# hustvl/4DGaussians

Hardware: NVIDIA H100
Metric: render FPS @300k gauss 1352x1014 (fused deform+rasterize forward); train-step ms in `train_step` (higher is better)
Workload: dtype f32

## Files before the change

### 4dgaussians_b200/csrc/g4d_deform_tc.cu

```cuda
#include "geom_finish.cuh"
#include "tc_wgmma.cuh"

namespace g4d {

template <int ARITH> struct TcArith;
template <> struct TcArith<2> {
    static constexpr int KS = 16, ES = 2, EPC = 8, NWG = 2, PH = 1;
    static constexpr float SF = 64.f, SA = 8.f, SW = 256.f;
};
template <> struct TcArith<1> {
    static constexpr int KS = 8, ES = 4, EPC = 4, NWG = 1, PH = 4;
    static constexpr float SF = 1.f, SA = 1.f, SW = 1.f;
};
constexpr float kF16Max = 65504.f;
constexpr int kStageCols = 60;
constexpr uint32_t kMaxSmemPerBlock = 227u * 1024u;
constexpr uint32_t kTcStaticSmem = (uint32_t)((sizeof(CameraDev) + 127) & ~(size_t)127);

struct TcSmem { uint32_t w1, w0, w2, bias, w2s, stage, bars, part_bytes, total; };

inline TcSmem tc_smem_layout(int arith, int F, bool sh) {
    const uint32_t es = arith == 2 ? 2u : 4u, ph = arith == 2 ? 1u : 4u, nwg = arith == 2 ? 2u : 1u;
    TcSmem s{};
    uint32_t off = 0;
// ... 99 lines not shown

template <int ARITH, int N, int NS, int NSP>
__device__ __forceinline__ void gemm3(float (&d)[N / 2], const Frags<NS>& a, int s0, uint32_t b_hi, uint32_t b_lo, uint32_t bcols,
                                      bool accumulate) {
    using A = TcArith<ARITH>;
    const uint64_t dh = wg::desc_kmajor(b_hi, bcols, A::EPC), dl = wg::desc_kmajor(b_lo, bcols, A::EPC);
    wg::fence_regs(d);
    wg::fence();
#pragma unroll
    for (int p = 0; p < 3; ++p) {
#pragma unroll
        for (int s = 0; s < NSP; ++s) {
            const uint64_t bd = ((p == 1) ? dl : dh) + (uint64_t)(16 * s);
            const uint32_t acc = (accumulate || p > 0 || s > 0) ? 1u : 0u;
            if constexpr (ARITH == 2) wg::mma_f16_rs<N, 0>(d, p == 0 ? a.lo[s0 + s] : a.hi[s0 + s], bd, acc);
            else wg::mma_tf32_rs<N>(d, p == 0 ? a.lo[s0 + s] : a.hi[s0 + s], bd, acc);
        }
    }
    wg::commit();
    wg::wait_all();
    wg::fence_regs(d);
}

template <int ARITH>
__device__ __forceinline__ void relu_to_frags(const float (&d)[64], float inv, const float* __restrict__ bias, int t, Frags<128 / TcArith<ARITH>::KS>& a,
                                              uint32_t (&b0)[4], uint32_t (&b1)[4], float& mx) {
#pragma unroll
    for (int w = 0; w < 4; ++w) { b0[w] = 0u; b1[w] = 0u; }
#pragma unroll
    for (int j = 0; j < 16; ++j) {
        const int c = 8 * j + 2 * t;
        const float2 bb = *reinterpret_cast<const float2*>(bias + c);
        const float x0 = fmaf(d[4 * j], inv, bb.x), x1 = fmaf(d[4 * j + 1], inv, bb.y);
        const float y0 = fmaf(d[4 * j + 2], inv, bb.x), y1 = fmaf(d[4 * j + 3], inv, bb.y);
        const int sh = 8 * (j & 3) + 2 * t;
        b0[j >> 2] |= ((x0 > 0.f ? 1u : 0u) | (x1 > 0.f ? 2u : 0u)) << sh;
        b1[j >> 2] |= ((y0 > 0.f ? 1u : 0u) | (y1 > 0.f ? 2u : 0u)) << sh;
        const float r0 = fmaxf(x0, 0.f), r1 = fmaxf(x1, 0.f), r2 = fmaxf(y0, 0.f), r3 = fmaxf(y1, 0.f);
        mx = fmaxf(mx, fmaxf(fmaxf(r0, r1), fmaxf(r2, r3)));
        put_block<ARITH>(a, j, r0, r1, r2, r3);
    }
#pragma unroll
    for (int w = 0; w < 4; ++w) {
        b0[w] |= __shfl_xor_sync(0xffffffffu, b0[w], 1); b0[w] |= __shfl_xor_sync(0xffffffffu, b0[w], 2);
        b1[w] |= __shfl_xor_sync(0xffffffffu, b1[w], 1); b1[w] |= __shfl_xor_sync(0xffffffffu, b1[w], 2);
    }
}

__device__ __forceinline__ void store_bits(uint32_t* base, int slot, int64_t n, int64_t g0, int64_t g1, int t, const uint32_t (&b0)[4],
                                           const uint32_t (&b1)[4]) {
    const uint32_t w0 = t == 0 ? b0[0] : t == 1 ? b0[1] : t == 2 ? b0[2] : b0[3];
    const uint32_t w1 = t == 0 ? b1[0] : t == 1 ? b1[1] : t == 2 ? b1[2] : b1[3];
    if (g0 < n) base[((size_t)slot * (size_t)n + (size_t)g0) * 4 + t] = w0;
    if (g1 < n) base[((size_t)slot * (size_t)n + (size_t)g1) * 4 + t] = w1;
}

__device__ __forceinline__ void mbar_arrive(void* bar) {
    asm volatile("mbarrier.arrive.shared::cta.b64 _, [%0];" ::"r"(smem_u32(bar)) : "memory");
}
__device__ __forceinline__ void bar_sync(int id, int count) { asm volatile("bar.sync %0, %1;" ::"r"(id), "r"(count) : "memory"); }

template <int ARITH, int MODE, int C, int L, bool SAVE>
__global__ void __launch_bounds__(TcArith<ARITH>::NWG * 128, 1)
deform_tc_kernel(DeformDesc d, TcWeights tw, TcSmem Ls, const CameraDev* __restrict__ camp, int use_cam, int64_t n, DeformIO io) {
    using A = TcArith<ARITH>;
    constexpr int F = C * L, NS0 = F / A::KS, NS1 = 128 / A::KS, NSP = NS1 / A::PH, TM = 64 * A::NWG, NT = 128 * A::NWG;
    static_assert(F % 16 == 0 && F <= 64, "feature width must be 32, 48 or 64");
    constexpr float kInvL0 = A::SA / (A::SF * A::SW), kInvH = 1.f / (A::SA * A::SW), kInvHS = 1.f / A::SW;
// ... 42 lines not shown
    uint32_t hseq = 0;
    {
        int k = 0;
        for (int h = 0; h < G4D_NUM_HEADS; ++h)
            if (d.head_mask & (1 << h)) hseq |= (uint32_t)h << (3 * k++);
    }
    const int64_t ntiles = (n + TM - 1) / TM;
    const int64_t my_tiles = (int64_t)blockIdx.x < ntiles ? (ntiles - 1 - blockIdx.x) / gridDim.x + 1 : 0;
    const uint32_t per_tile = (uint32_t)(m_heads * A::PH), total_items = (uint32_t)my_tiles * per_tile;
    auto issue = [&](uint32_t u) {
        const uint32_t s = u & 1u, r = u % per_tile;
        if (u >= 2) mbar_wait(bar_empty + s, ((u >> 1) - 1u) & 1u);
        const int h = (int)((hseq >> (3 * (r / A::PH))) & 7u);
        mbar_expect_tx(bar_full + s, Ls.part_bytes);
        tma_bulk_g2s(smem + Ls.w1 + s * Ls.part_bytes, reinterpret_cast<const uint8_t*>(tw.w1[h]) + (r % A::PH) * Ls.part_bytes,
                     Ls.part_bytes, bar_full + s);
    };
    if (tid == 0) {
        const uint32_t w0b = 2u * 128u * F * A::ES, w2b = hsh ? 2u * 48u * 128u * A::ES : 0u;
        mbar_expect_tx(bar_w0, w0b + w2b);
        tma_bulk_g2s(smem + Ls.w0, tw.w0, w0b, bar_w0);
        if (hsh) tma_bulk_g2s(smem + Ls.w2, tw.w2[4], w2b, bar_w0);
        if (total_items) issue(0);
    }
    __syncwarp();
    mbar_wait(bar_w0, 0);
    const uint32_t sW0 = wg::smem_addr(smem + Ls.w0), sW1 = wg::smem_addr(smem + Ls.w1), sW2 = wg::smem_addr(smem + Ls.w2);
    const float* b2s = sBias + 128 + G4D_NUM_HEADS * 128;
    float mx = 0.f;
    uint32_t u = 0;
    const bool dbg = tw.dbg && tid == 0;
    const long long t_start = dbg ? clock64() : 0;
    long long t_wait = 0;

    for (int64_t it = 0; it < my_tiles; ++it) {
        const int64_t tile = (int64_t)blockIdx.x + it * gridDim.x;
        const int64_t row0 = tile * TM + wgi * 64, g0 = row0 + r0, g1 = row0 + r1;
        float acc[64];
        {
            Frags<NS0> x;
            const float* f0 = tw.feat + g0 * F;
            const float* f1 = tw.feat + g1 * F;
#pragma unroll
            for (int s = 0; s < NS0; ++s) {
                float v[8];
#pragma unroll
                for (int hlf = 0; hlf < 2; ++hlf) {
                    const int c = ARITH == 2 ? 16 * s + 8 * hlf + 2 * t : 8 * s + 4 * hlf + t;
                    if (ARITH == 2) {
                        const float2 p0 = g0 < n ? __ldg(reinterpret_cast<const float2*>(f0 + c)) : make_float2(0.f, 0.f);
                        const float2 p1 = g1 < n ? __ldg(reinterpret_cast<const float2*>(f1 + c)) : make_float2(0.f, 0.f);
                        v[4 * hlf] = p0.x * A::SF; v[4 * hlf + 1] = p0.y * A::SF; v[4 * hlf + 2] = p1.x * A::SF; v[4 * hlf + 3] = p1.y * A::SF;
                    } else {
                        v[4 * hlf] = g0 < n ? __ldg(f0 + c) : 0.f;
                        v[4 * hlf + 2] = g1 < n ? __ldg(f1 + c) : 0.f;
                    }
                }
                if (ARITH == 2) {
#pragma unroll
                    for (int e = 0; e < 8; ++e) mx = fmaxf(mx, fabsf(v[e]));
                    wg::f16_split2(v[0], v[1], x.hi[s][0], x.lo[s][0]);
                    wg::f16_split2(v[2], v[3], x.hi[s][1], x.lo[s][1]);
                    wg::f16_split2(v[4], v[5], x.hi[s][2], x.lo[s][2]);
                    wg::f16_split2(v[6], v[7], x.hi[s][3], x.lo[s][3]);
                } else {
                    wg::tf32_split(v[0], x.hi[s][0], x.lo[s][0]);
                    wg::tf32_split(v[2], x.hi[s][1], x.lo[s][1]);
                    wg::tf32_split(v[4], x.hi[s][2], x.lo[s][2]);
                    wg::tf32_split(v[6], x.hi[s][3], x.lo[s][3]);
                }
            }
            gemm3<ARITH, 128, NS0, NS0>(acc, x, 0, sW0, sW0 + 128u * F * A::ES, F, false);
        }
        Frags<NS1> a1;
        {
            uint32_t bw0[4], bw1[4];
            relu_to_frags<ARITH>(acc, kInvL0, sBias, t, a1, bw0, bw1, mx);
            if (SAVE) store_bits(tw.relu_bits, 0, n, g0, g1, t, bw0, bw1);
        }
        if (t == 0) {
#pragma unroll
            for (int j = 0; j < 11; ++j) { stage[r0 * kStageCols + j] = 0.f; stage[r1 * kStageCols + j] = 0.f; }
        }
#pragma unroll 1
        for (int k = 0; k < m_heads; ++k) {
            const int h = (int)((hseq >> (3 * k)) & 7u);
#pragma unroll 1
            for (int p = 0; p < A::PH; ++p, ++u) {
                if (tid == 0 && u + 1 < total_items) issue(u + 1);
                __syncwarp();
                const uint32_t s = u & 1u;
                const long long t0 = dbg ? clock64() : 0;
                mbar_wait(bar_full + s, (u >> 1) & 1u);
                if (dbg) t_wait += clock64() - t0;
                const uint32_t b = sW1 + s * Ls.part_bytes;
                if constexpr (A::PH == 1) {
                    gemm3<ARITH, 128, NS1, NSP>(acc, a1, 0, b, b + Ls.part_bytes / 2, 128 / A::PH, false);
                } else {
#pragma unroll
                    for (int pp = 0; pp < A::PH; ++pp)
                        if (pp == p) gemm3<ARITH, 128, NS1, NSP>(acc, a1, pp * NSP, b, b + Ls.part_bytes / 2, 128 / A::PH, pp != 0);
                }
                if (lane == 0) mbar_arrive(bar_empty + s);
            }
            uint32_t bw0[4], bw1[4];
            if (h < 4) {
                const float* b1 = sBias + 128 + h * 128;
                const float4* w2 = sW2s + h * 128;
                float o0[4] = {0.f, 0.f, 0.f, 0.f}, o1[4] = {0.f, 0.f, 0.f, 0.f};
#pragma unroll
                for (int w = 0; w < 4; ++w) { bw0[w] = 0u; bw1[w] = 0u; }
#pragma unroll
                for (int j = 0; j < 16; ++j) {
                    const int c = 8 * j + 2 * t;
                    const float2 bb = *reinterpret_cast<const float2*>(b1 + c);
                    const float x0 = fmaf(acc[4 * j], kInvH, bb.x), x1 = fmaf(acc[4 * j + 1], kInvH, bb.y);
                    const float y0 = fmaf(acc[4 * j + 2], kInvH, bb.x), y1 = fmaf(acc[4 * j + 3], kInvH, bb.y);
                    const int sh = 8 * (j & 3) + 2 * t;
                    bw0[j >> 2] |= ((x0 > 0.f ? 1u : 0u) | (x1 > 0.f ? 2u : 0u)) << sh;
                    bw1[j >> 2] |= ((y0 > 0.f ? 1u : 0u) | (y1 > 0.f ? 2u : 0u)) << sh;
                    const float4 wa = w2[c], wb = w2[c + 1];
                    const float ax = fmaxf(x0, 0.f), ay = fmaxf(x1, 0.f), bx = fmaxf(y0, 0.f), by = fmaxf(y1, 0.f);
                    o0[0] = fmaf(ay, wb.x, fmaf(ax, wa.x, o0[0])); o0[1] = fmaf(ay, wb.y, fmaf(ax, wa.y, o0[1]));
                    o0[2] = fmaf(ay, wb.z, fmaf(ax, wa.z, o0[2])); o0[3] = fmaf(ay, wb.w, fmaf(ax, wa.w, o0[3]));
                    o1[0] = fmaf(by, wb.x, fmaf(bx, wa.x, o1[0])); o1[1] = fmaf(by, wb.y, fmaf(bx, wa.y, o1[1]));
                    o1[2] = fmaf(by, wb.z, fmaf(bx, wa.z, o1[2])); o1[3] = fmaf(by, wb.w, fmaf(bx, wa.w, o1[3]));
                }
#pragma unroll
                for (int o = 0; o < 4; ++o) {
                    o0[o] += __shfl_xor_sync(0xffffffffu, o0[o], 1); o0[o] += __shfl_xor_sync(0xffffffffu, o0[o], 2);
                    o1[o] += __shfl_xor_sync(0xffffffffu, o1[o], 1); o1[o] += __shfl_xor_sync(0xffffffffu, o1[o], 2);
                }
#pragma unroll
                for (int w = 0; w < 4; ++w) {
                    bw0[w] |= __shfl_xor_sync(0xffffffffu, bw0[w], 1); bw0[w] |= __shfl_xor_sync(0xffffffffu, bw0[w], 2);
                    bw1[w] |= __shfl_xor_sync(0xffffffffu, bw1[w], 1); bw1[w] |= __shfl_xor_sync(0xffffffffu, bw1[w], 2);
                }
                if (t == 0) {
                    const int ko = head_out(h), col = head_col(h);
#pragma unroll
                    for (int o = 0; o < 4; ++o) {
                        if (o < ko) {
                            stage[r0 * kStageCols + col + o] = o0[o] + b2s[4 * h + o];
                            stage[r1 * kStageCols + col + o] = o1[o] + b2s[4 * h + o];
                        }
                    }
                }
            } else {
                relu_to_frags<ARITH>(acc, kInvHS, sBias + 128 + 4 * 128, t, a1, bw0, bw1, mx);
                float acc2[24];
                gemm3<ARITH, 48, NS1, NS1>(acc2, a1, 0, sW2, sW2 + 48u * 128u * A::ES, 128, false);
                const float* b2sh = b2s + 16;
#pragma unroll
                for (int j = 0; j < 6; ++j) {
                    const int c = 8 * j + 2 * t;
                    stage[r0 * kStageCols + 11 + c] = fmaf(acc2[4 * j], kInvH, b2sh[c]);
                    stage[r0 * kStageCols + 12 + c] = fmaf(acc2[4 * j + 1], kInvH, b2sh[c + 1]);
                    stage[r1 * kStageCols + 11 + c] = fmaf(acc2[4 * j + 2], kInvH, b2sh[c]);
                    stage[r1 * kStageCols + 12 + c] = fmaf(acc2[4 * j + 3], kInvH, b2sh[c + 1]);
                }
            }
            if (SAVE) store_bits(tw.relu_bits, 1 + h, n, g0, g1, t, bw0, bw1);
        }
        bar_sync(1 + wgi, 128);
        {
            const int row = t128 & 63;
            const int64_t gi = row0 + row;
            const float* o = stage + row * kStageCols;
            if (gi < n) {
                const Vec3 p{io.xyz[3 * gi] + o[0], io.xyz[3 * gi + 1] + o[1], io.xyz[3 * gi + 2] + o[2]};
                if (t128 < 64) {
                    float sl[3] = {0.f, 0.f, 0.f}, q[4] = {0.f, 0.f, 0.f, 0.f}, ol = 0.f;
                    if (io.scaling) { sl[0] = io.scaling[3 * gi]; sl[1] = io.scaling[3 * gi + 1]; sl[2] = io.scaling[3 * gi + 2]; }
                    if (io.rotation) { const float4 r4 = *reinterpret_cast<const float4*>(io.rotation + 4 * gi); q[0] = r4.x; q[1] = r4.y; q[2] = r4.z; q[3] = r4.w; }
                    if (io.opacity) ol = io.opacity[gi];
                    sl[0] += o[3]; sl[1] += o[4]; sl[2] += o[5];
                    q[0] += o[6]; q[1] += o[7]; q[2] += o[8]; q[3] += o[9];
                    ol += o[10];
                    if (MODE == 0) {
                        io.out_xyz[3 * gi] = p.x; io.out_xyz[3 * gi + 1] = p.y; io.out_xyz[3 * gi + 2] = p.z;
                        if (io.out_scaling) { io.out_scaling[3 * gi] = sl[0]; io.out_scaling[3 * gi + 1] = sl[1]; io.out_scaling[3 * gi + 2] = sl[2]; }
                        if (io.out_rotation) *reinterpret_cast<float4*>(io.out_rotation + 4 * gi) = make_float4(q[0], q[1], q[2], q[3]);
                        if (io.out_opacity) io.out_opacity[gi] = ol;
                    } else {
                        fused_finish_geometry(cam, io, gi, p, sl, q, ol);
                    }
                } else {
                    float dsh[48];
#pragma unroll
                    for (int j = 0; j < 48; ++j) dsh[j] = hsh ? o[11 + j] : 0.f;
                    if (MODE == 0) {
                        if (io.out_shs && hsh) {
#pragma unroll
                            for (int j = 0; j < 48; j += 4) {
                                const float4 b = *reinterpret_cast<const float4*>(io.shs + gi * 48 + j);
                                *reinterpret_cast<float4*>(io.out_shs + gi * 48 + j) = make_float4(b.x + dsh[j], b.y + dsh[j + 1], b.z + dsh[j + 2], b.w + dsh[j + 3]);
                            }
                        }
                    } else {
                        fused_finish_colour(cam, io, gi, p, hsh, dsh);
                    }
                }
            }
        }
        bar_sync(1 + wgi, 128);
    }
    if (ARITH == 2 && mx >= kF16Max && tw.status) *reinterpret_cast<volatile uint32_t*>(tw.status) = 1u;
    if (dbg) { tw.dbg[blockIdx.x * 12] = clock64() - t_start; tw.dbg[blockIdx.x * 12 + 1] = t_wait; }
}

template <int C4>
__global__ void __launch_bounds__(256) deform_features_kernel(DeformDesc d, int64_t n, const float* __restrict__ xyz, float* __restrict__ feat) {
    pdl_wait();
    pdl_trigger();
    const int64_t t = (int64_t)blockIdx.x * 256 + threadIdx.x;
    const int64_t g = t / C4;
    const int v = (int)(t % C4);
    if (g >= n) return;
    const AabbNorm nrm(d.aabb);
    float pcs[3];
#pragma unroll
    for (int a = 0; a < 3; ++a) pcs[a] = nrm(a, xyz[3 * g + a]);
    for (int l = 0; l < d.levels; ++l) {
        Tap1D tx[3];
#pragma unroll
        for (int a = 0; a < 3; ++a) tx[a] = make_tap(pcs[a], d.res[l][a]);
        *reinterpret_cast<float4*>(feat + g * d.F + l * d.C + 4 * v) = sample_vector(d.planes[l], d.trow[l], d.res[l], tx, v, C4);
    }
}

cudaError_t launch_deform_features(const DeformDesc& d, int64_t n, const float* xyz, float* feat, bool pdl, cudaStream_t st) {
// ... 59 lines not shown
```

### 4dgaussians_b200/csrc/tc_wgmma.cuh

```cuda
#pragma once
#include <cuda_runtime.h>
#include <stdint.h>

namespace g4d {
namespace wg {

__device__ __forceinline__ uint32_t smem_addr(const void* p) { return (uint32_t)__cvta_generic_to_shared(p); }

__device__ __forceinline__ uint64_t make_desc(uint32_t saddr, uint32_t lbo_bytes, uint32_t sbo_bytes) {
    return (uint64_t)((saddr >> 4) & 0x3FFFu) | ((uint64_t)((lbo_bytes >> 4) & 0x3FFFu) << 16) |
           ((uint64_t)((sbo_bytes >> 4) & 0x3FFFu) << 32);
}
__device__ __forceinline__ uint64_t desc_kmajor(uint32_t saddr, uint32_t cols, uint32_t elems_per_core) {
    return make_desc(saddr, 128u, (cols / elems_per_core) * 128u);
}
__device__ __forceinline__ uint64_t desc_mnmajor(uint32_t saddr, uint32_t cols) { return make_desc(saddr, (cols / 8u) * 128u, 128u); }

__host__ __device__ constexpr uint32_t img16_off(uint32_t row, uint32_t col, uint32_t ncols) {
    return (row >> 3) * ((ncols >> 3) * 128u) + (col >> 3) * 128u + (row & 7u) * 16u + (col & 7u) * 2u;
}
__host__ __device__ constexpr uint32_t img32_off(uint32_t row, uint32_t col, uint32_t ncols) {
    return (row >> 3) * ((ncols >> 2) * 128u) + (col >> 2) * 128u + (row & 7u) * 16u + (col & 3u) * 4u;
}
__host__ __device__ constexpr uint32_t tf32_kperm(uint32_t c) { return (c & ~7u) | ((c & 1u) ? 4u + ((c & 7u) >> 1) : ((c & 7u) >> 1)); }

__device__ __forceinline__ void fence() { asm volatile("wgmma.fence.sync.aligned;" ::: "memory"); }
__device__ __forceinline__ void commit() { asm volatile("wgmma.commit_group.sync.aligned;" ::: "memory"); }
__device__ __forceinline__ void wait_all() { asm volatile("wgmma.wait_group.sync.aligned 0;" ::: "memory"); }
__device__ __forceinline__ void fence_proxy_async() { asm volatile("fence.proxy.async.shared::cta;" ::: "memory"); }
template <int M>
__device__ __forceinline__ void fence_regs(float (&d)[M]) {
#pragma unroll
    for (int i = 0; i < M; ++i) asm volatile("" : "+f"(d[i])::"memory");
}
template <int M>
__device__ __forceinline__ void fence_regs(uint32_t (&d)[M]) {
#pragma unroll
    for (int i = 0; i < M; ++i) asm volatile("" : "+r"(d[i])::"memory");
}

__device__ __forceinline__ uint32_t tf32_rna(float x) {
    uint32_t r;
    asm("cvt.rna.tf32.f32 %0, %1;" : "=r"(r) : "f"(x));
    return r;
}
__device__ __forceinline__ void tf32_split(float x, uint32_t& hi, uint32_t& lo) {
    hi = tf32_rna(x);
    lo = tf32_rna(x - __uint_as_float(hi));
}
__device__ __forceinline__ uint16_t bf16_rn(float x) {
    uint16_t r;
// ... 15 lines not shown
    asm("{\n\t.reg .b16 l, h;\n\tmov.b32 {l, h}, %2;\n\tcvt.f32.f16 %0, l;\n\tcvt.f32.f16 %1, h;\n\t}" : "=f"(ha), "=f"(hb) : "r"(hi));
    asm("cvt.rn.satfinite.f16x2.f32 %0, %1, %2;" : "=r"(lo) : "f"(b - hb), "f"(a - ha));
}

template <int NS>
struct Frags { uint32_t hi[NS][4], lo[NS][4]; };


__device__ __forceinline__ void mma_tf32_rs_n16(float (&d)[8], const uint32_t (&a)[4], uint64_t b, uint32_t acc) {
    asm volatile(
        "{\n.reg .pred p;\nsetp.ne.b32 p, %13, 0;\n"
        "wgmma.mma_async.sync.aligned.m64n16k8.f32.tf32.tf32 {%0, %1, %2, %3, %4, %5, %6, %7}, {%8, %9, %10, %11}, %12, p, 1, 1;\n}\n"
        : "+f"(d[0]), "+f"(d[1]), "+f"(d[2]), "+f"(d[3]), "+f"(d[4]), "+f"(d[5]), "+f"(d[6]), "+f"(d[7])
        : "r"(a[0]), "r"(a[1]), "r"(a[2]), "r"(a[3]), "l"(b), "r"(acc));
}

__device__ __forceinline__ void mma_tf32_rs_n48(float (&d)[24], const uint32_t (&a)[4], uint64_t b, uint32_t acc) {
    asm volatile(
        "{\n.reg .pred p;\nsetp.ne.b32 p, %29, 0;\n"
        "wgmma.mma_async.sync.aligned.m64n48k8.f32.tf32.tf32 {%0, %1, %2, %3, %4, %5, %6, %7, %8, %9, %10, %11, %12, %13, %14, %15, %16, %17, %18, %19, %20, %21, %22, %23}, {%24, %25, %26, %27}, %28, p, 1, 1;\n}\n"
        : "+f"(d[0]), "+f"(d[1]), "+f"(d[2]), "+f"(d[3]), "+f"(d[4]), "+f"(d[5]), "+f"(d[6]), "+f"(d[7]),
          "+f"(d[8]), "+f"(d[9]), "+f"(d[10]), "+f"(d[11]), "+f"(d[12]), "+f"(d[13]), "+f"(d[14]), "+f"(d[15]),
          "+f"(d[16]), "+f"(d[17]), "+f"(d[18]), "+f"(d[19]), "+f"(d[20]), "+f"(d[21]), "+f"(d[22]), "+f"(d[23])
        : "r"(a[0]), "r"(a[1]), "r"(a[2]), "r"(a[3]), "l"(b), "r"(acc));
}

__device__ __forceinline__ void mma_tf32_rs_n128(float (&d)[64], const uint32_t (&a)[4], uint64_t b, uint32_t acc) {
    asm volatile(
        "{\n.reg .pred p;\nsetp.ne.b32 p, %69, 0;\n"
        "wgmma.mma_async.sync.aligned.m64n128k8.f32.tf32.tf32 {%0, %1, %2, %3, %4, %5, %6, %7, %8, %9, %10, %11, %12, %13, %14, %15, %16, %17, %18, %19, %20, %21, %22, %23, %24, %25, %26, %27, %28, %29, %30, %31, %32, %33, %34, %35, %36, %37, %38, %39, %40, %41, %42, %43, %44, %45, %46, %47, %48, %49, %50, %51, %52, %53, %54, %55, %56, %57, %58, %59, %60, %61, %62, %63}, {%64, %65, %66, %67}, %68, p, 1, 1;\n}\n"
        : "+f"(d[0]), "+f"(d[1]), "+f"(d[2]), "+f"(d[3]), "+f"(d[4]), "+f"(d[5]), "+f"(d[6]), "+f"(d[7]),
          "+f"(d[8]), "+f"(d[9]), "+f"(d[10]), "+f"(d[11]), "+f"(d[12]), "+f"(d[13]), "+f"(d[14]), "+f"(d[15]),
          "+f"(d[16]), "+f"(d[17]), "+f"(d[18]), "+f"(d[19]), "+f"(d[20]), "+f"(d[21]), "+f"(d[22]), "+f"(d[23]),
          "+f"(d[24]), "+f"(d[25]), "+f"(d[26]), "+f"(d[27]), "+f"(d[28]), "+f"(d[29]), "+f"(d[30]), "+f"(d[31]),
          "+f"(d[32]), "+f"(d[33]), "+f"(d[34]), "+f"(d[35]), "+f"(d[36]), "+f"(d[37]), "+f"(d[38]), "+f"(d[39]),
          "+f"(d[40]), "+f"(d[41]), "+f"(d[42]), "+f"(d[43]), "+f"(d[44]), "+f"(d[45]), "+f"(d[46]), "+f"(d[47]),
          "+f"(d[48]), "+f"(d[49]), "+f"(d[50]), "+f"(d[51]), "+f"(d[52]), "+f"(d[53]), "+f"(d[54]), "+f"(d[55]),
          "+f"(d[56]), "+f"(d[57]), "+f"(d[58]), "+f"(d[59]), "+f"(d[60]), "+f"(d[61]), "+f"(d[62]), "+f"(d[63])
        : "r"(a[0]), "r"(a[1]), "r"(a[2]), "r"(a[3]), "l"(b), "r"(acc));
}

template <int N>
__device__ __forceinline__ void mma_tf32_rs(float (&d)[N / 2], const uint32_t (&a)[4], uint64_t b, uint32_t acc) {
    static_assert(N == 16 || N == 48 || N == 128, "unsupported N");
    if constexpr (N == 16) mma_tf32_rs_n16(d, a, b, acc);
    else if constexpr (N == 48) mma_tf32_rs_n48(d, a, b, acc);
    else if constexpr (N == 128) mma_tf32_rs_n128(d, a, b, acc);
}

template <int TB>
__device__ __forceinline__ void mma_f16_rs_n16(float (&d)[8], const uint32_t (&a)[4], uint64_t b, uint32_t acc) {
    asm volatile(
        "{\n.reg .pred p;\nsetp.ne.b32 p, %13, 0;\n"
        "wgmma.mma_async.sync.aligned.m64n16k16.f32.f16.f16 {%0, %1, %2, %3, %4, %5, %6, %7}, {%8, %9, %10, %11}, %12, p, 1, 1, %14;\n}\n"
        : "+f"(d[0]), "+f"(d[1]), "+f"(d[2]), "+f"(d[3]), "+f"(d[4]), "+f"(d[5]), "+f"(d[6]), "+f"(d[7])
        : "r"(a[0]), "r"(a[1]), "r"(a[2]), "r"(a[3]), "l"(b), "r"(acc), "n"(TB));
}

template <int TB>
__device__ __forceinline__ void mma_f16_rs_n48(float (&d)[24], const uint32_t (&a)[4], uint64_t b, uint32_t acc) {
    asm volatile(
        "{\n.reg .pred p;\nsetp.ne.b32 p, %29, 0;\n"
        "wgmma.mma_async.sync.aligned.m64n48k16.f32.f16.f16 {%0, %1, %2, %3, %4, %5, %6, %7, %8, %9, %10, %11, %12, %13, %14, %15, %16, %17, %18, %19, %20, %21, %22, %23}, {%24, %25, %26, %27}, %28, p, 1, 1, %30;\n}\n"
        : "+f"(d[0]), "+f"(d[1]), "+f"(d[2]), "+f"(d[3]), "+f"(d[4]), "+f"(d[5]), "+f"(d[6]), "+f"(d[7]),
          "+f"(d[8]), "+f"(d[9]), "+f"(d[10]), "+f"(d[11]), "+f"(d[12]), "+f"(d[13]), "+f"(d[14]), "+f"(d[15]),
          "+f"(d[16]), "+f"(d[17]), "+f"(d[18]), "+f"(d[19]), "+f"(d[20]), "+f"(d[21]), "+f"(d[22]), "+f"(d[23])
        : "r"(a[0]), "r"(a[1]), "r"(a[2]), "r"(a[3]), "l"(b), "r"(acc), "n"(TB));
}

template <int TB>
__device__ __forceinline__ void mma_f16_rs_n128(float (&d)[64], const uint32_t (&a)[4], uint64_t b, uint32_t acc) {
    asm volatile(
        "{\n.reg .pred p;\nsetp.ne.b32 p, %69, 0;\n"
        "wgmma.mma_async.sync.aligned.m64n128k16.f32.f16.f16 {%0, %1, %2, %3, %4, %5, %6, %7, %8, %9, %10, %11, %12, %13, %14, %15, %16, %17, %18, %19, %20, %21, %22, %23, %24, %25, %26, %27, %28, %29, %30, %31, %32, %33, %34, %35, %36, %37, %38, %39, %40, %41, %42, %43, %44, %45, %46, %47, %48, %49, %50, %51, %52, %53, %54, %55, %56, %57, %58, %59, %60, %61, %62, %63}, {%64, %65, %66, %67}, %68, p, 1, 1, %70;\n}\n"
        : "+f"(d[0]), "+f"(d[1]), "+f"(d[2]), "+f"(d[3]), "+f"(d[4]), "+f"(d[5]), "+f"(d[6]), "+f"(d[7]),
          "+f"(d[8]), "+f"(d[9]), "+f"(d[10]), "+f"(d[11]), "+f"(d[12]), "+f"(d[13]), "+f"(d[14]), "+f"(d[15]),
          "+f"(d[16]), "+f"(d[17]), "+f"(d[18]), "+f"(d[19]), "+f"(d[20]), "+f"(d[21]), "+f"(d[22]), "+f"(d[23]),
          "+f"(d[24]), "+f"(d[25]), "+f"(d[26]), "+f"(d[27]), "+f"(d[28]), "+f"(d[29]), "+f"(d[30]), "+f"(d[31]),
          "+f"(d[32]), "+f"(d[33]), "+f"(d[34]), "+f"(d[35]), "+f"(d[36]), "+f"(d[37]), "+f"(d[38]), "+f"(d[39]),
          "+f"(d[40]), "+f"(d[41]), "+f"(d[42]), "+f"(d[43]), "+f"(d[44]), "+f"(d[45]), "+f"(d[46]), "+f"(d[47]),
          "+f"(d[48]), "+f"(d[49]), "+f"(d[50]), "+f"(d[51]), "+f"(d[52]), "+f"(d[53]), "+f"(d[54]), "+f"(d[55]),
          "+f"(d[56]), "+f"(d[57]), "+f"(d[58]), "+f"(d[59]), "+f"(d[60]), "+f"(d[61]), "+f"(d[62]), "+f"(d[63])
        : "r"(a[0]), "r"(a[1]), "r"(a[2]), "r"(a[3]), "l"(b), "r"(acc), "n"(TB));
}

template <int N, int TB>
__device__ __forceinline__ void mma_f16_rs(float (&d)[N / 2], const uint32_t (&a)[4], uint64_t b, uint32_t acc) {
    static_assert(N == 16 || N == 48 || N == 128, "unsupported N");
    if constexpr (N == 16) mma_f16_rs_n16<TB>(d, a, b, acc);
    else if constexpr (N == 48) mma_f16_rs_n48<TB>(d, a, b, acc);
    else if constexpr (N == 128) mma_f16_rs_n128<TB>(d, a, b, acc);
}

template <int TB>
__device__ __forceinline__ void mma_bf16_rs_n16(float (&d)[8], const uint32_t (&a)[4], uint64_t b, uint32_t acc) {
    asm volatile(
        "{\n.reg .pred p;\nsetp.ne.b32 p, %13, 0;\n"
        "wgmma.mma_async.sync.aligned.m64n16k16.f32.bf16.bf16 {%0, %1, %2, %3, %4, %5, %6, %7}, {%8, %9, %10, %11}, %12, p, 1, 1, %14;\n}\n"
        : "+f"(d[0]), "+f"(d[1]), "+f"(d[2]), "+f"(d[3]), "+f"(d[4]), "+f"(d[5]), "+f"(d[6]), "+f"(d[7])
        : "r"(a[0]), "r"(a[1]), "r"(a[2]), "r"(a[3]), "l"(b), "r"(acc), "n"(TB));
}

template <int TB>
__device__ __forceinline__ void mma_bf16_rs_n32(float (&d)[16], const uint32_t (&a)[4], uint64_t b, uint32_t acc) {
    asm volatile(
        "{\n.reg .pred p;\nsetp.ne.b32 p, %21, 0;\n"
        "wgmma.mma_async.sync.aligned.m64n32k16.f32.bf16.bf16 {%0, %1, %2, %3, %4, %5, %6, %7, %8, %9, %10, %11, %12, %13, %14, %15}, {%16, %17, %18, %19}, %20, p, 1, 1, %22;\n}\n"
        : "+f"(d[0]), "+f"(d[1]), "+f"(d[2]), "+f"(d[3]), "+f"(d[4]), "+f"(d[5]), "+f"(d[6]), "+f"(d[7]),
          "+f"(d[8]), "+f"(d[9]), "+f"(d[10]), "+f"(d[11]), "+f"(d[12]), "+f"(d[13]), "+f"(d[14]), "+f"(d[15])
        : "r"(a[0]), "r"(a[1]), "r"(a[2]), "r"(a[3]), "l"(b), "r"(acc), "n"(TB));
}

template <int TB>
// ... 129 lines not shown
```

Measured before the change: 904.9.

## Split deform MLP wgmma into N-halves and overlap epilogues with async MMA

Each 128-wide wgmma is split into two 64-column halves committed as separate groups, so the ReLU and small-head epilogue of one half runs while the other half's MMA is still in flight. The next head's first half is issued before the previous head's second half is post-processed. Weight staging moves to a two-ahead TMA prefetch, and the f16 non-save path prefetches the next tile's features into registers during the current tile. This adds register pressure and more complex wait_group and barrier ordering, which risks spills or hazards.

```diff
diff --git a/4dgaussians_b200/csrc/g4d_deform_tc.cu b/4dgaussians_b200/csrc/g4d_deform_tc.cu
--- a/4dgaussians_b200/csrc/g4d_deform_tc.cu
+++ b/4dgaussians_b200/csrc/g4d_deform_tc.cu
@@ -145,17 +145,51 @@
     wg::fence_regs(d);
 }
 
-template <int ARITH>
-__device__ __forceinline__ void relu_to_frags(const float (&d)[64], float inv, const float* __restrict__ bias, int t, Frags<128 / TcArith<ARITH>::KS>& a,
-                                              uint32_t (&b0)[4], uint32_t (&b1)[4], float& mx) {
-#pragma unroll
-    for (int w = 0; w < 4; ++w) { b0[w] = 0u; b1[w] = 0u; }
-#pragma unroll
-    for (int j = 0; j < 16; ++j) {
-        const int c = 8 * j + 2 * t;
+
+template <int ARITH, int NS, int NSP>
+__device__ __forceinline__ void issue_half(float (&d)[32], const Frags<NS>& a, int s0, uint32_t b_hi, uint32_t b_lo, uint32_t bcols,
+                                           int half, bool accumulate) {
+    using A = TcArith<ARITH>;
+    const uint32_t off = (uint32_t)half * 8u * (bcols / A::EPC) * 128u;
+    const uint64_t dh = wg::desc_kmajor(b_hi + off, bcols, A::EPC), dl = wg::desc_kmajor(b_lo + off, bcols, A::EPC);
+    wg::fence_regs(d);
+    wg::fence();
+#pragma unroll
+    for (int p = 0; p < 3; ++p) {
+#pragma unroll
+        for (int s = 0; s < NSP; ++s) {
+            const uint64_t bd = ((p == 1) ? dl : dh) + (uint64_t)(16 * s);
+            const uint32_t acc = (accumulate || p > 0 || s > 0) ? 1u : 0u;
+            if constexpr (ARITH == 2) wg::mma_f16_rs<64, 0>(d, p == 0 ? a.lo[s0 + s] : a.hi[s0 + s], bd, acc);
+            else wg::mma_tf32_rs<64>(d, p == 0 ? a.lo[s0 + s] : a.hi[s0 + s], bd, acc);
+        }
+    }
+    wg::commit();
+}
+
+template <int N>
+__device__ __forceinline__ void retire(float (&d)[32]) {
+    wg::wait_group<N>();
+    wg::fence_regs(d);
+}
+
+template <int NS>
+__device__ __forceinline__ void fence_frags(Frags<NS>& a) {
+#pragma unroll
+    for (int s = 0; s < NS; ++s) { wg::fence_regs(a.hi[s]); wg::fence_regs(a.lo[s]); }
+}
+
+template <int ARITH, int HALF>
+__device__ __forceinline__ void relu_half(const float (&d)[32], float inv, const float* __restrict__ bias, int t, Frags<128 / TcArith<ARITH>::KS>& a,
+                                          uint32_t (&b0)[4], uint32_t (&b1)[4], float& mx) {
+#pragma unroll
+    for (int w = 2 * HALF; w < 2 * HALF + 2; ++w) { b0[w] = 0u; b1[w] = 0u; }
+#pragma unroll
+    for (int i = 0; i < 8; ++i) {
+        const int j = 8 * HALF + i, c = 8 * j + 2 * t;
         const float2 bb = *reinterpret_cast<const float2*>(bias + c);
-        const float x0 = fmaf(d[4 * j], inv, bb.x), x1 = fmaf(d[4 * j + 1], inv, bb.y);
-        const float y0 = fmaf(d[4 * j + 2], inv, bb.x), y1 = fmaf(d[4 * j + 3], inv, bb.y);
+        const float x0 = fmaf(d[4 * i], inv, bb.x), x1 = fmaf(d[4 * i + 1], inv, bb.y);
+        const float y0 = fmaf(d[4 * i + 2], inv, bb.x), y1 = fmaf(d[4 * i + 3], inv, bb.y);
         const int sh = 8 * (j & 3) + 2 * t;
         b0[j >> 2] |= ((x0 > 0.f ? 1u : 0u) | (x1 > 0.f ? 2u : 0u)) << sh;
         b1[j >> 2] |= ((y0 > 0.f ? 1u : 0u) | (y1 > 0.f ? 2u : 0u)) << sh;
@@ -164,9 +198,60 @@
         put_block<ARITH>(a, j, r0, r1, r2, r3);
     }
 #pragma unroll
-    for (int w = 0; w < 4; ++w) {
+    for (int w = 2 * HALF; w < 2 * HALF + 2; ++w) {
         b0[w] |= __shfl_xor_sync(0xffffffffu, b0[w], 1); b0[w] |= __shfl_xor_sync(0xffffffffu, b0[w], 2);
         b1[w] |= __shfl_xor_sync(0xffffffffu, b1[w], 1); b1[w] |= __shfl_xor_sync(0xffffffffu, b1[w], 2);
+    }
+}
+
+template <int HALF>
+__device__ __forceinline__ void small_head_half(const float (&d)[32], float inv, const float* __restrict__ b1, const float4* __restrict__ w2,
+                                                int t, float (&o0)[4], float (&o1)[4], uint32_t (&bw0)[4], uint32_t (&bw1)[4]) {
+    if (HALF == 0) {
+#pragma unroll
+        for (int o = 0; o < 4; ++o) { o0[o] = 0.f; o1[o] = 0.f; }
+    }
+#pragma unroll
+    for (int w = 2 * HALF; w < 2 * HALF + 2; ++w) { bw0[w] = 0u; bw1[w] = 0u; }
+#pragma unroll
+    for (int i = 0; i < 8; ++i) {
+        const int j = 8 * HALF + i, c = 8 * j + 2 * t;
+        const float2 bb = *reinterpret_cast<const float2*>(b1 + c);
+        const float x0 = fmaf(d[4 * i], inv, bb.x), x1 = fmaf(d[4 * i + 1], inv, bb.y);
+        const float y0 = fmaf(d[4 * i + 2], inv, bb.x), y1 = fmaf(d[4 * i + 3], inv, bb.y);
+        const int sh = 8 * (j & 3) + 2 * t;
+        bw0[j >> 2] |= ((x0 > 0.f ? 1u : 0u) | (x1 > 0.f ? 2u : 0u)) << sh;
+        bw1[j >> 2] |= ((y0 > 0.f ? 1u : 0u) | (y1 > 0.f ? 2u : 0u)) << sh;
+        const float4 wa = w2[c], wb = w2[c + 1];
+        const float ax = fmaxf(x0, 0.f), ay = fmaxf(x1, 0.f), bx = fmaxf(y0, 0.f), by = fmaxf(y1, 0.f);
+        o0[0] = fmaf(ay, wb.x, fmaf(ax, wa.x, o0[0])); o0[1] = fmaf(ay, wb.y, fmaf(ax, wa.y, o0[1]));
+        o0[2] = fmaf(ay, wb.z, fmaf(ax, wa.z, o0[2])); o0[3] = fmaf(ay, wb.w, fmaf(ax, wa.w, o0[3]));
+        o1[0] = fmaf(by, wb.x, fmaf(bx, wa.x, o1[0])); o1[1] = fmaf(by, wb.y, fmaf(bx, wa.y, o1[1]));
+        o1[2] = fmaf(by, wb.z, fmaf(bx, wa.z, o1[2])); o1[3] = fmaf(by, wb.w, fmaf(bx, wa.w, o1[3]));
+    }
+#pragma unroll
+    for (int w = 2 * HALF; w < 2 * HALF + 2; ++w) {
+        bw0[w] |= __shfl_xor_sync(0xffffffffu, bw0[w], 1); bw0[w] |= __shfl_xor_sync(0xffffffffu, bw0[w], 2);
+        bw1[w] |= __shfl_xor_sync(0xffffffffu, bw1[w], 1); bw1[w] |= __shfl_xor_sync(0xffffffffu, bw1[w], 2);
+    }
+}
+
+__device__ __forceinline__ void small_head_out(float (&o0)[4], float (&o1)[4], const float* __restrict__ b2, int h, float* stage, int r0,
+                                               int r1, int t) {
+#pragma unroll
+    for (int o = 0; o < 4; ++o) {
+        o0[o] += __shfl_xor_sync(0xffffffffu, o0[o], 1); o0[o] += __shfl_xor_sync(0xffffffffu, o0[o], 2);
+        o1[o] += __shfl_xor_sync(0xffffffffu, o1[o], 1); o1[o] += __shfl_xor_sync(0xffffffffu, o1[o], 2);
+    }
+    if (t == 0) {
+        const int ko = head_out(h), col = head_col(h);
+#pragma unroll
+        for (int o = 0; o < 4; ++o) {
+            if (o < ko) {
+                stage[r0 * kStageCols + col + o] = o0[o] + b2[4 * h + o];
+                stage[r1 * kStageCols + col + o] = o1[o] + b2[4 * h + o];
+            }
+        }
     }
 }
 
@@ -255,6 +340,7 @@
         tma_bulk_g2s(smem + Ls.w0, tw.w0, w0b, bar_w0);
         if (hsh) tma_bulk_g2s(smem + Ls.w2, tw.w2[4], w2b, bar_w0);
         if (total_items) issue(0);
+        if (total_items > 1) issue(1);
     }
     __syncwarp();
     mbar_wait(bar_w0, 0);
@@ -264,31 +350,57 @@
     uint32_t u = 0;
     const bool dbg = tw.dbg && tid == 0;
     const long long t_start = dbg ? clock64() : 0;
-    long long t_wait = 0;
+    long long t_wait = 0, t_exp = 0, t_ret = 0;
+    auto release = [&](uint32_t v) {
+        if (lane == 0) mbar_arrive(bar_empty + (v & 1u));
+        if (tid == 0 && v + 2 < total_items) issue(v + 2);
+        __syncwarp();
+    };
+    auto wait_w1 = [&](uint32_t v) {
+        const long long t0 = dbg ? clock64() : 0;
+        mbar_wait(bar_full + (v & 1u), (v >> 1) & 1u);
+        if (dbg) t_wait += clock64() - t0;
+        return sW1 + (v & 1u) * Ls.part_bytes;
+    };
+
+    constexpr bool kPrefetch = ARITH == 2 && !SAVE;
+    float fv[NS0][8];
+    auto load_feat = [&](int64_t tile) {
+        const int64_t h0 = tile * TM + wgi * 64 + r0, h1 = h0 + 8;
+        const float* f0 = tw.feat + h0 * F;
+        const float* f1 = tw.feat + h1 * F;
+#pragma unroll
+        for (int s = 0; s < NS0; ++s) {
+#pragma unroll
+            for (int hlf = 0; hlf < 2; ++hlf) {
+                const int c = ARITH == 2 ? 16 * s + 8 * hlf + 2 * t : 8 * s + 4 * hlf + t;
+                if (ARITH == 2) {
+                    const float2 p0 = h0 < n ? __ldg(reinterpret_cast<const float2*>(f0 + c)) : make_float2(0.f, 0.f);
+                    const float2 p1 = h1 < n ? __ldg(reinterpret_cast<const float2*>(f1 + c)) : make_float2(0.f, 0.f);
+                    fv[s][4 * hlf] = p0.x; fv[s][4 * hlf + 1] = p0.y; fv[s][4 * hlf + 2] = p1.x; fv[s][4 * hlf + 3] = p1.y;
+                } else {
+                    fv[s][4 * hlf] = h0 < n ? __ldg(f0 + c) : 0.f;
+                    fv[s][4 * hlf + 2] = h1 < n ? __ldg(f1 + c) : 0.f;
+                }
+            }
+        }
+    };
+    if (kPrefetch && my_tiles > 0) load_feat(blockIdx.x);
 
     for (int64_t it = 0; it < my_tiles; ++it) {
         const int64_t tile = (int64_t)blockIdx.x + it * gridDim.x;
         const int64_t row0 = tile * TM + wgi * 64, g0 = row0 + r0, g1 = row0 + r1;
-        float acc[64];
+        float accA[32], accB[32];
+        Frags<NS1> a1;
+        uint32_t bw0[4], bw1[4];
+        if (!kPrefetch) load_feat(tile);
         {
             Frags<NS0> x;
-            const float* f0 = tw.feat + g0 * F;
-            const float* f1 = tw.feat + g1 * F;
 #pragma unroll
             for (int s = 0; s < NS0; ++s) {
                 float v[8];
 #pragma unroll
-                for (int hlf = 0; hlf < 2; ++hlf) {
-                    const int c = ARITH == 2 ? 16 * s + 8 * hlf + 2 * t : 8 * s + 4 * hlf + t;
-                    if (ARITH == 2) {
-                        const float2 p0 = g0 < n ? __ldg(reinterpret_cast<const float2*>(f0 + c)) : make_float2(0.f, 0.f);
-                        const float2 p1 = g1 < n ? __ldg(reinterpret_cast<const float2*>(f1 + c)) : make_float2(0.f, 0.f);
-                        v[4 * hlf] = p0.x * A::SF; v[4 * hlf + 1] = p0.y * A::SF; v[4 * hlf + 2] = p1.x * A::SF; v[4 * hlf + 3] = p1.y * A::SF;
-                    } else {
-                        v[4 * hlf] = g0 < n ? __ldg(f0 + c) : 0.f;
-                        v[4 * hlf + 2] = g1 < n ? __ldg(f1 + c) : 0.f;
-                    }
-                }
+                for (int e = 0; e < 8; ++e) v[e] = ARITH == 2 ? fv[s][e] * A::SF : fv[s][e];
                 if (ARITH == 2) {
 #pragma unroll
                     for (int e = 0; e < 8; ++e) mx = fmaxf(mx, fabsf(v[e]));
@@ -303,98 +415,91 @@
                     wg::tf32_split(v[6], x.hi[s][3], x.lo[s][3]);
                 }
             }
-            gemm3<ARITH, 128, NS0, NS0>(acc, x, 0, sW0, sW0 + 128u * F * A::ES, F, false);
-        }
-        Frags<NS1> a1;
-        {
-            uint32_t bw0[4], bw1[4];
-            relu_to_frags<ARITH>(acc, kInvL0, sBias, t, a1, bw0, bw1, mx);
-            if (SAVE) store_bits(tw.relu_bits, 0, n, g0, g1, t, bw0, bw1);
-        }
+            issue_half<ARITH, NS0, NS0>(accA, x, 0, sW0, sW0 + 128u * F * A::ES, F, 0, false);
+            issue_half<ARITH, NS0, NS0>(accB, x, 0, sW0, sW0 + 128u * F * A::ES, F, 1, false);
+            retire<1>(accA);
+            relu_half<ARITH, 0>(accA, kInvL0, sBias, t, a1, bw0, bw1, mx);
+            retire<0>(accB);
+            fence_frags(x);
+        }
+        relu_half<ARITH, 1>(accB, kInvL0, sBias, t, a1, bw0, bw1, mx);
+        if (SAVE) store_bits(tw.relu_bits, 0, n, g0, g1, t, bw0, bw1);
         if (t == 0) {
 #pragma unroll
             for (int j = 0; j < 11; ++j) { stage[r0 * kStageCols + j] = 0.f; stage[r1 * kStageCols + j] = 0.f; }
         }
+        float o0[4], o1[4];
+        if (m_heads > 0) {
+            int k = 0;
+#pragma unroll
+            for (int p = 0; p < A::PH; ++p, ++u) {
+                const uint32_t b = wait_w1(u);
+                issue_half<ARITH, NS1, NSP>(accA, a1, p * NSP, b, b + Ls.part_bytes / 2, 128 / A::PH, 0, p != 0);
+                issue_half<ARITH, NS1, NSP>(accB, a1, p * NSP, b, b + Ls.part_bytes / 2, 128 / A::PH, 1, p != 0);
+                if (p + 1 < A::PH) {
+                    retire<0>(accB);
+                    wg::fence_regs(accA);
+                    release(u);
+                }
+            }
 #pragma unroll 1
-        for (int k = 0; k < m_heads; ++k) {
-            const int h = (int)((hseq >> (3 * k)) & 7u);
-#pragma unroll 1
-            for (int p = 0; p < A::PH; ++p, ++u) {
-                if (tid == 0 && u + 1 < total_items) issue(u + 1);
-                __syncwarp();
-                const uint32_t s = u & 1u;
-                const long long t0 = dbg ? clock64() : 0;
-                mbar_wait(bar_full + s, (u >> 1) & 1u);
-                if (dbg) t_wait += clock64() - t0;
-                const uint32_t b = sW1 + s * Ls.part_bytes;
-                if constexpr (A::PH == 1) {
-                    gemm3<ARITH, 128, NS1, NSP>(acc, a1, 0, b, b + Ls.part_bytes / 2, 128 / A::PH, false);
-                } else {
-#pragma unroll
-                    for (int pp = 0; pp < A::PH; ++pp)
-                        if (pp == p) gemm3<ARITH, 128, NS1, NSP>(acc, a1, pp * NSP, b, b + Ls.part_bytes / 2, 128 / A::PH, pp != 0);
+            for (;;) {
+                const int h = (int)((hseq >> (3 * k)) & 7u);
+                if (h == 4) {
+                    retire<0>(accB);
+                    wg::fence_regs(accA);
+                    if (dbg) t_ret = clock64();
+                    release(u - 1);
+                    relu_half<ARITH, 0>(accA, kInvHS, sBias + 128 + 4 * 128, t, a1, bw0, bw1, mx);
+                    relu_half<ARITH, 1>(accB, kInvHS, sBias + 128 + 4 * 128, t, a1, bw0, bw1, mx);
+                    if (dbg) t_exp += clock64() - t_ret;
+                    float acc2[24];
+                    gemm3<ARITH, 48, NS1, NS1>(acc2, a1, 0, sW2, sW2 + 48u * 128u * A::ES, 128, false);
+                    const float* b2sh = b2s + 16;
+#pragma unroll
+                    for (int j = 0; j < 6; ++j) {
+                        const int c = 8 * j + 2 * t;
+                        stage[r0 * kStageCols + 11 + c] = fmaf(acc2[4 * j], kInvH, b2sh[c]);
+                        stage[r0 * kStageCols + 12 + c] = fmaf(acc2[4 * j + 1], kInvH, b2sh[c + 1]);
+                        stage[r1 * kStageCols + 11 + c] = fmaf(acc2[4 * j + 2], kInvH, b2sh[c]);
+                        stage[r1 * kStageCols + 12 + c] = fmaf(acc2[4 * j + 3], kInvH, b2sh[c + 1]);
+                    }
+                    if (SAVE) store_bits(tw.relu_bits, 1 + 4, n, g0, g1, t, bw0, bw1);
+                    break;
                 }
-                if (lane == 0) mbar_arrive(bar_empty + s);
-            }
-            uint32_t bw0[4], bw1[4];
-            if (h < 4) {
-                const float* b1 = sBias + 128 + h * 128;
-                const float4* w2 = sW2s + h * 128;
-                float o0[4] = {0.f, 0.f, 0.f, 0.f}, o1[4] = {0.f, 0.f, 0.f, 0.f};
-#pragma unroll
-                for (int w = 0; w < 4; ++w) { bw0[w] = 0u; bw1[w] = 0u; }
-#pragma unroll
-                for (int j = 0; j < 16; ++j) {
-                    const int c = 8 * j + 2 * t;
-                    const float2 bb = *reinterpret_cast<const float2*>(b1 + c);
-                    const float x0 = fmaf(acc[4 * j], kInvH, bb.x), x1 = fmaf(acc[4 * j + 1], kInvH, bb.y);
-                    const float y0 = fmaf(acc[4 * j + 2], kInvH, bb.x), y1 = fmaf(acc[4 * j + 3], kInvH, bb.y);
-                    const int sh = 8 * (j & 3) + 2 * t;
-                    bw0[j >> 2] |= ((x0 > 0.f ? 1u : 0u) | (x1 > 0.f ? 2u : 0u)) << sh;
-                    bw1[j >> 2] |= ((y0 > 0.f ? 1u : 0u) | (y1 > 0.f ? 2u : 0u)) << sh;
-                    const float4 wa = w2[c], wb = w2[c + 1];
-                    const float ax = fmaxf(x0, 0.f), ay = fmaxf(x1, 0.f), bx = fmaxf(y0, 0.f), by = fmaxf(y1, 0.f);
-                    o0[0] = fmaf(ay, wb.x, fmaf(ax, wa.x, o0[0])); o0[1] = fmaf(ay, wb.y, fmaf(ax, wa.y, o0[1]));
-                    o0[2] = fmaf(ay, wb.z, fmaf(ax, wa.z, o0[2])); o0[3] = fmaf(ay, wb.w, fmaf(ax, wa.w, o0[3]));
-                    o1[0] = fmaf(by, wb.x, fmaf(bx, wa.x, o1[0])); o1[1] = fmaf(by, wb.y, fmaf(bx, wa.y, o1[1]));
-                    o1[2] = fmaf(by, wb.z, fmaf(bx, wa.z, o1[2])); o1[3] = fmaf(by, wb.w, fmaf(bx, wa.w, o1[3]));
+                retire<1>(accA);
+                small_head_half<0>(accA, kInvH, sBias + 128 + h * 128, sW2s + h * 128, t, o0, o1, bw0, bw1);
+                if (++k == m_heads) {
+                    retire<0>(accB);
+                    if (dbg) t_ret = clock64();
+                    release(u - 1);
+                    small_head_half<1>(accB, kInvH, sBias + 128 + h * 128, sW2s + h * 128, t, o0, o1, bw0, bw1);
+                    small_head_out(o0, o1, b2s, h, stage, r0, r1, t);
+                    if (SAVE) store_bits(tw.relu_bits, 1 + h, n, g0, g1, t, bw0, bw1);
+                    if (dbg) t_exp += clock64() - t_ret;
+                    break;
                 }
 #pragma unroll
-                for (int o = 0; o < 4; ++o) {
-                    o0[o] += __shfl_xor_sync(0xffffffffu, o0[o], 1); o0[o] += __shfl_xor_sync(0xffffffffu, o0[o], 2);
-                    o1[o] += __shfl_xor_sync(0xffffffffu, o1[o], 1); o1[o] += __shfl_xor_sync(0xffffffffu, o1[o], 2);
-                }
-#pragma unroll
-                for (int w = 0; w < 4; ++w) {
-                    bw0[w] |= __shfl_xor_sync(0xffffffffu, bw0[w], 1); bw0[w] |= __shfl_xor_sync(0xffffffffu, bw0[w], 2);
-                    bw1[w] |= __shfl_xor_sync(0xffffffffu, bw1[w], 1); bw1[w] |= __shfl_xor_sync(0xffffffffu, bw1[w], 2);
-                }
-                if (t == 0) {
-                    const int ko = head_out(h), col = head_col(h);
-#pragma unroll
-                    for (int o = 0; o < 4; ++o) {
-                        if (o < ko) {
-                            stage[r0 * kStageCols + col + o] = o0[o] + b2s[4 * h + o];
-                            stage[r1 * kStageCols + col + o] = o1[o] + b2s[4 * h + o];
-                        }
+                for (int p = 0; p < A::PH; ++p, ++u) {
+                    const uint32_t b = wait_w1(u);
+                    issue_half<ARITH, NS1, NSP>(accA, a1, p * NSP, b, b + Ls.part_bytes / 2, 128 / A::PH, 0, p != 0);
+                    if (p == 0) {
+                        retire<1>(accB);
+                        release(u - 1);
+                        small_head_half<1>(accB, kInvH, sBias + 128 + h * 128, sW2s + h * 128, t, o0, o1, bw0, bw1);
+                        small_head_out(o0, o1, b2s, h, stage, r0, r1, t);
+                        if (SAVE) store_bits(tw.relu_bits, 1 + h, n, g0, g1, t, bw0, bw1);
+                    }
+                    issue_half<ARITH, NS1, NSP>(accB, a1, p * NSP, b, b + Ls.part_bytes / 2, 128 / A::PH, 1, p != 0);
+                    if (p + 1 < A::PH) {
+                        retire<0>(accB);
+                        wg::fence_regs(accA);
+                        release(u);
                     }
                 }
-            } else {
-                relu_to_frags<ARITH>(acc, kInvHS, sBias + 128 + 4 * 128, t, a1, bw0, bw1, mx);
-                float acc2[24];
-                gemm3<ARITH, 48, NS1, NS1>(acc2, a1, 0, sW2, sW2 + 48u * 128u * A::ES, 128, false);
-                const float* b2sh = b2s + 16;
-#pragma unroll
-                for (int j = 0; j < 6; ++j) {
-                    const int c = 8 * j + 2 * t;
-                    stage[r0 * kStageCols + 11 + c] = fmaf(acc2[4 * j], kInvH, b2sh[c]);
-                    stage[r0 * kStageCols + 12 + c] = fmaf(acc2[4 * j + 1], kInvH, b2sh[c + 1]);
-                    stage[r1 * kStageCols + 11 + c] = fmaf(acc2[4 * j + 2], kInvH, b2sh[c]);
-                    stage[r1 * kStageCols + 12 + c] = fmaf(acc2[4 * j + 3], kInvH, b2sh[c + 1]);
-                }
             }
-            if (SAVE) store_bits(tw.relu_bits, 1 + h, n, g0, g1, t, bw0, bw1);
-        }
+        }
+        if (kPrefetch && it + 1 < my_tiles) load_feat(tile + gridDim.x);
         bar_sync(1 + wgi, 128);
         {
             const int row = t128 & 63;
@@ -439,7 +544,7 @@
         bar_sync(1 + wgi, 128);
     }
     if (ARITH == 2 && mx >= kF16Max && tw.status) *reinterpret_cast<volatile uint32_t*>(tw.status) = 1u;
-    if (dbg) { tw.dbg[blockIdx.x * 12] = clock64() - t_start; tw.dbg[blockIdx.x * 12 + 1] = t_wait; }
+    if (dbg) { tw.dbg[blockIdx.x * 12] = clock64() - t_start; tw.dbg[blockIdx.x * 12 + 1] = t_wait; tw.dbg[blockIdx.x * 12 + 2] = t_exp; }
 }
 
 template <int C4>
diff --git a/4dgaussians_b200/csrc/tc_wgmma.cuh b/4dgaussians_b200/csrc/tc_wgmma.cuh
--- a/4dgaussians_b200/csrc/tc_wgmma.cuh
+++ b/4dgaussians_b200/csrc/tc_wgmma.cuh
@@ -27,6 +27,8 @@
 __device__ __forceinline__ void fence() { asm volatile("wgmma.fence.sync.aligned;" ::: "memory"); }
 __device__ __forceinline__ void commit() { asm volatile("wgmma.commit_group.sync.aligned;" ::: "memory"); }
 __device__ __forceinline__ void wait_all() { asm volatile("wgmma.wait_group.sync.aligned 0;" ::: "memory"); }
+template <int N>
+__device__ __forceinline__ void wait_group() { asm volatile("wgmma.wait_group.sync.aligned %0;" ::"n"(N) : "memory"); }
 __device__ __forceinline__ void fence_proxy_async() { asm volatile("fence.proxy.async.shared::cta;" ::: "memory"); }
 template <int M>
 __device__ __forceinline__ void fence_regs(float (&d)[M]) {
@@ -88,6 +90,17 @@
         : "+f"(d[0]), "+f"(d[1]), "+f"(d[2]), "+f"(d[3]), "+f"(d[4]), "+f"(d[5]), "+f"(d[6]), "+f"(d[7]),
           "+f"(d[8]), "+f"(d[9]), "+f"(d[10]), "+f"(d[11]), "+f"(d[12]), "+f"(d[13]), "+f"(d[14]), "+f"(d[15]),
           "+f"(d[16]), "+f"(d[17]), "+f"(d[18]), "+f"(d[19]), "+f"(d[20]), "+f"(d[21]), "+f"(d[22]), "+f"(d[23])
+        : "r"(a[0]), "r"(a[1]), "r"(a[2]), "r"(a[3]), "l"(b), "r"(acc));
+}
+
+__device__ __forceinline__ void mma_tf32_rs_n64(float (&d)[32], const uint32_t (&a)[4], uint64_t b, uint32_t acc) {
+    asm volatile(
+        "{\n.reg .pred p;\nsetp.ne.b32 p, %37, 0;\n"
+        "wgmma.mma_async.sync.aligned.m64n64k8.f32.tf32.tf32 {%0, %1, %2, %3, %4, %5, %6, %7, %8, %9, %10, %11, %12, %13, %14, %15, %16, %17, %18, %19, %20, %21, %22, %23, %24, %25, %26, %27, %28, %29, %30, %31}, {%32, %33, %34, %35}, %36, p, 1, 1;\n}\n"
+        : "+f"(d[0]), "+f"(d[1]), "+f"(d[2]), "+f"(d[3]), "+f"(d[4]), "+f"(d[5]), "+f"(d[6]), "+f"(d[7]),
+          "+f"(d[8]), "+f"(d[9]), "+f"(d[10]), "+f"(d[11]), "+f"(d[12]), "+f"(d[13]), "+f"(d[14]), "+f"(d[15]),
+          "+f"(d[16]), "+f"(d[17]), "+f"(d[18]), "+f"(d[19]), "+f"(d[20]), "+f"(d[21]), "+f"(d[22]), "+f"(d[23]),
+          "+f"(d[24]), "+f"(d[25]), "+f"(d[26]), "+f"(d[27]), "+f"(d[28]), "+f"(d[29]), "+f"(d[30]), "+f"(d[31])
         : "r"(a[0]), "r"(a[1]), "r"(a[2]), "r"(a[3]), "l"(b), "r"(acc));
 }
 
@@ -108,9 +121,10 @@
 
 template <int N>
 __device__ __forceinline__ void mma_tf32_rs(float (&d)[N / 2], const uint32_t (&a)[4], uint64_t b, uint32_t acc) {
-    static_assert(N == 16 || N == 48 || N == 128, "unsupported N");
+    static_assert(N == 16 || N == 48 || N == 64 || N == 128, "unsupported N");
     if constexpr (N == 16) mma_tf32_rs_n16(d, a, b, acc);
     else if constexpr (N == 48) mma_tf32_rs_n48(d, a, b, acc);
+    else if constexpr (N == 64) mma_tf32_rs_n64(d, a, b, acc);
     else if constexpr (N == 128) mma_tf32_rs_n128(d, a, b, acc);
 }
 
@@ -131,6 +145,18 @@
         : "+f"(d[0]), "+f"(d[1]), "+f"(d[2]), "+f"(d[3]), "+f"(d[4]), "+f"(d[5]), "+f"(d[6]), "+f"(d[7]),
           "+f"(d[8]), "+f"(d[9]), "+f"(d[10]), "+f"(d[11]), "+f"(d[12]), "+f"(d[13]), "+f"(d[14]), "+f"(d[15]),
           "+f"(d[16]), "+f"(d[17]), "+f"(d[18]), "+f"(d[19]), "+f"(d[20]), "+f"(d[21]), "+f"(d[22]), "+f"(d[23])
+        : "r"(a[0]), "r"(a[1]), "r"(a[2]), "r"(a[3]), "l"(b), "r"(acc), "n"(TB));
+}
+
+template <int TB>
+__device__ __forceinline__ void mma_f16_rs_n64(float (&d)[32], const uint32_t (&a)[4], uint64_t b, uint32_t acc) {
+    asm volatile(
+        "{\n.reg .pred p;\nsetp.ne.b32 p, %37, 0;\n"
+        "wgmma.mma_async.sync.aligned.m64n64k16.f32.f16.f16 {%0, %1, %2, %3, %4, %5, %6, %7, %8, %9, %10, %11, %12, %13, %14, %15, %16, %17, %18, %19, %20, %21, %22, %23, %24, %25, %26, %27, %28, %29, %30, %31}, {%32, %33, %34, %35}, %36, p, 1, 1, %38;\n}\n"
+        : "+f"(d[0]), "+f"(d[1]), "+f"(d[2]), "+f"(d[3]), "+f"(d[4]), "+f"(d[5]), "+f"(d[6]), "+f"(d[7]),
+          "+f"(d[8]), "+f"(d[9]), "+f"(d[10]), "+f"(d[11]), "+f"(d[12]), "+f"(d[13]), "+f"(d[14]), "+f"(d[15]),
+          "+f"(d[16]), "+f"(d[17]), "+f"(d[18]), "+f"(d[19]), "+f"(d[20]), "+f"(d[21]), "+f"(d[22]), "+f"(d[23]),
+          "+f"(d[24]), "+f"(d[25]), "+f"(d[26]), "+f"(d[27]), "+f"(d[28]), "+f"(d[29]), "+f"(d[30]), "+f"(d[31])
         : "r"(a[0]), "r"(a[1]), "r"(a[2]), "r"(a[3]), "l"(b), "r"(acc), "n"(TB));
 }
 
@@ -152,9 +178,10 @@
 
 template <int N, int TB>
 __device__ __forceinline__ void mma_f16_rs(float (&d)[N / 2], const uint32_t (&a)[4], uint64_t b, uint32_t acc) {
-    static_assert(N == 16 || N == 48 || N == 128, "unsupported N");
+    static_assert(N == 16 || N == 48 || N == 64 || N == 128, "unsupported N");
     if constexpr (N == 16) mma_f16_rs_n16<TB>(d, a, b, acc);
     else if constexpr (N == 48) mma_f16_rs_n48<TB>(d, a, b, acc);
+    else if constexpr (N == 64) mma_f16_rs_n64<TB>(d, a, b, acc);
     else if constexpr (N == 128) mma_f16_rs_n128<TB>(d, a, b, acc);
 }
 
```

Result: faster. 914.2 (median of 6 runs) (+1.0%).
